# igorauad/gr-dvbs2rx

Hardware: AMD Instinct MI355X
Metric: FECFRAMEs/sec (coded Gbit/s) @ 50 LDPC iters, QPSK 1/2 normal (higher is better)
Workload: dtype int8; 1 GPU; QPSK 1/2 normal FECFRAME (DVB_S2_TABLE_B4, N=64800), 50 LDPC iterations cap, batch=4096 frames per GPU, group G=32, input=noise; frames_per_gpu=4096, max_trials=50, group_size=32, parallelism=frames sharded over 1 GPU(s), no collective

## Files before the change

### gr-dvbs2rx_amd/csrc/ldpc_kernel.hpp

```cpp
#pragma once
#include <hip/hip_runtime.h>
#include <cstdint>
#include "demap_math.hpp"
#include "ldpc_launch.h"
#include "ldpc_prims.hpp"
#include "ldpc_node_plain.hpp"
#include "ldpc_node_packed.hpp"
#include "ldpc_node_hazard.hpp"

namespace dvbs2 {

#define DVBS2_DEG_CASE(D) case D: if constexpr (D >= 3 && D <= DMAX && D > DMAX - 8) { \
        { if (layer0) check_node<(D >= 3 ? D : 3), true, false, false, TC>(lds_all, ent, jj, lb, mw, nm); else { if constexpr (!kPure) check_node<(D >= 3 ? D : 3), false, false, false, TC>(lds_all, ent, jj, lb, mw, nm); } } } else DVBS2_NM_CLEAR break;
#define DVBS2_DEG_SWITCH switch (deg) { DVBS2_DEGREES_3_32(DVBS2_DEG_CASE) default: DVBS2_NM_CLEAR break; }

#define DVBS2_V2_CASE(D) case D: if constexpr (D >= 3 && D <= DMAX && D > DMAX - 8) { check_node_v2<(D >= 3 ? D : 3), DMAX, TC>(ent, jj + lb, mw, nm, prefetch); } else DVBS2_NM_CLEAR break;
#define DVBS2_V2_SWITCH switch (deg) { DVBS2_DEGREES_3_32(DVBS2_V2_CASE) default: DVBS2_NM_CLEAR break; }
#define DVBS2_NM_CLEAR { _Pragma("unroll") for (int w_ = 0; w_ < MW; w_++) nm[w_] = 0u; }
#define DVBS2_RUN_CASE(D) case D - 2: if constexpr (D >= 3 && D <= DMAX && D > DMAX - 8) { run(std::integral_constant<int, (D >= 3 ? D : 3)>{}); } break;

#define DVBS2_CHAIN_CASE(D) case D: if constexpr (D >= 4 && D <= DMAX && D > DMAX - 8) { check_node_chain_v2<(D >= 4 ? D : 4), DMAX, TC>(ent, jj, jj + lb, work, block, mw, nm, htab16, hb_ctr, hb_epoch, hb_lane); } break;
#define DVBS2_CHAIN_SWITCH switch (deg) { DVBS2_DEGREES_4_32(DVBS2_CHAIN_CASE) default: break; }

#define DVBS2_HAZ_NODE(D, NCV, ...) \
// ... 135 lines not shown
            if (dm.mode == 1) {
                const float scalar = qpsk_scalar(N0);
                for (int sidx = tid; sidx < dm.n_syms; sidx += kHalf) {
                    const float2 v = src[sidx];
                    put(2 * sidx, qpsk_llr(v.x, scalar)); put(2 * sidx + 1, qpsk_llr(v.y, scalar));
                }
            } else {
                const float dp = psk8_dist_prec(N0);
                for (int sidx = tid; sidx < dm.n_syms; sidx += kHalf) {
                    const float2 v = src[sidx];
                    int8_t b0, b1, b2;
                    psk8_llr(v.x, v.y, dm.rr, dm.ri, dp, b0, b1, b2);
                    put(dm.ra0 + sidx, b0); put(dm.ra1 + sidx, b1); put(dm.ra2 + sidx, b2);
                }
            }
        } else if (fresh) {
            const uint2* src = reinterpret_cast<const uint2*>(llr_in + (size_t)f * N);
            for (int c = tid; c < N / 8; c += kHalf) {
                uint2 v = src[c];
                if constexpr (!TC) { v.x ^= 0x80808080u; v.y ^= 0x80808080u; }
                const int n = 8 * c;
                if (n < K) *reinterpret_cast<lds_v2u_t*>(lds + n) = (v2u32){ v.x, v.y };
                else {
                    int r = n - K;
                    int jq = r / q, iq = r - jq * q;
#pragma unroll
                    for (int b = 0; b < 8; b++) {
                        lds[K + kM * iq + jq] = (uint8_t)((b < 4 ? v.x >> (8 * b) : v.y >> (8 * (b - 4))) & 0xffu);
                        if (++iq == q) { iq = 0; ++jq; }
                    }
                }
            }
        } else {
            it = iters[f];
            if (it >= tgt) finished = true;
            else {
                const uint2* src = reinterpret_cast<const uint2*>(state + (size_t)f * N);
                for (int c = tid; c < N / 8; c += kHalf) { const uint2 v = src[c]; *reinterpret_cast<lds_v2u_t*>(lds + 8 * c) = (v2u32){ v.x ^ kObState, v.y ^ kObState }; }
            }
        }
    }
    const bool untouched = finished;
    if (tid == 0) { flags[0] = 0; flags[2] = 0; flags[3] = 0; flags[1] = finished ? 1 : 0; flags[4] = 0; }
    constexpr bool soft_bar = SOFT;
    volatile lds_i32_t* hb_ctr = soft_bar ? flags + 4 : nullptr;
    int hb_epoch = 0;
    const int hb_lane = lane;
    __syncthreads();
    TSTAMP(tB); tm_load = tB - tA;

    uint32_t* msg_base = msgs + (size_t)(have_frame ? f : 0) * q * MW * kMsgStride;
    const __amdgpu_buffer_rsrc_t mrs = __builtin_amdgcn_make_buffer_rsrc(msg_base, 0, q * MW * kMsgStride * 4, 0x00020000);
    constexpr int kLayerBytes = MW * kMsgStride * 4;
#define MSG_LD(soff, w, r4) __builtin_amdgcn_raw_buffer_load_b32(mrs, (r4), (soff) + (w) * (kMsgStride * 4), 0)
#define MSG_ST(v, soff, w, r4) __builtin_amdgcn_raw_buffer_store_b32((v), mrs, (r4), (soff) + (w) * (kMsgStride * 4), 0)
    auto msg_load = [&](uint32_t* dst, int soff, int r4) {
#pragma unroll
        for (int w = 0; w < MW; w++) dst[w] = MSG_LD(soff, w, r4);
    };
    auto msg_store = [&](const uint32_t* src, int soff, int r4) {
#pragma unroll
        for (int w = 0; w < MW; w++) MSG_ST(src[w], soff, w, r4);
    };
    auto take_msgs = [&](uint32_t* mw, uint32_t* pre, bool zero, uint32_t zero_word, int next, int r4) {
#pragma unroll
        for (int w = 0; w < MW; w++) mw[w] = pre[w];
        if (zero) {
            asm volatile("" ::: "memory");
#pragma unroll
            for (int w = 0; w < MW; w++) mw[w] = zero_word;
        } else msg_load(pre, next, r4);
    };
    bool is_good = false;

    for (;;) {
        TSTAMP(tS0);
        const bool need_synd = !finished && ((stop_on_good & 1) || it >= tgt);
        if (need_synd && active) {
            const int i0 = it % q;
            const uint32_t* rec = recs + (size_t)i0 * RS;
            const int deg = (int)(rec[0] & 0xffu) + 2;
            uint32_t x = 0, z = 0;
            constexpr bool kPretestChunk = DMAX != 16 && !(DMAX == 32 && SOFT);
            if constexpr (kPretestChunk) {
            for (int k0 = 0; k0 < deg; k0 += 4) {
                uint32_t e[8], v[4];
#pragma unroll
                for (int u = 0; u < 8; u++) e[u] = rec[4 + 2 * k0 + u];
#pragma unroll
                for (int u = 0; u < 4; u++) {
                    const int a0 = tid + (int)e[2 * u] - ((uint32_t)tid < e[2 * u + 1] ? 0 : kM);
                    v[u] = (uint32_t)lds[k0 + u < deg ? a0 : tid];
                }
#pragma unroll
                for (int u = 0; u < 4; u++) {
                    uint32_t w = v[u] ^ (TC ? 0x80u : 0x00u);
                    if (i0 == 0 && k0 + u == deg - 1 && tid == 0) w = 0x81u;
                    if (k0 + u < deg) { x ^= w; z |= (w == 0x80u); }
                }
            }
            } else
            for (int k = 0; k < deg; k++) {
                const int a0 = tid + (int)rec[4 + 2 * k] - ((uint32_t)tid < rec[5 + 2 * k] ? 0 : kM);
                uint32_t v = (uint32_t)lds[a0] ^ (TC ? 0x80u : 0x00u);
                if (i0 == 0 && k == deg - 1 && tid == 0) v = 0x81u;
                x ^= v;
                z |= (v == 0x80u);
            }
            const int bad_pre = (int)((((x >> 7) ^ (uint32_t)deg) & 1u) | z);
            if (__ballot(bad_pre) != 0 && lane == 0) flags[2] = 1;
        }
        lds_barrier();
        const bool need_full = need_synd && flags[2] == 0;
        if (tid == 0) flags[3] = need_full ? 1 : 0;
        lds_barrier();
        const bool full_any = flags[3] != 0 || (!soft_bar && !SOLO && other_flags[3] != 0);
        if (full_any) {
        if (need_full) {
            {
                const int zero = syndrome_sign_vectors(lds, sv, N, tid, TC);
                if (__ballot(zero != 0) != 0 && lane == 0) flags[0] = 1;
            }
        }
        TSTAMP(tC); tm_s1 += tC - tS0;
// ... 7 lines not shown
        lds_barrier();
        if (need_full) {
            int bad = 0;
            for (int item = tid; item < q * 12; item += kHalf) {
                const int i = item / 12, w = item - 12 * i;
                const uint32_t* rec = recs + (size_t)i * RS;
                const int deg = (int)(rec[0] & 0xffu) + 2;
                uint32_t e0[DMAX], e1[DMAX];
#pragma unroll
                for (int k = 0; k < DMAX; k++) { e0[k] = rec[4 + 2 * k]; e1[k] = rec[5 + 2 * k]; }
                uint32_t acc = 0;
#pragma unroll
                for (int k = 0; k < DMAX; k++) {
                    if (k < deg) {
                        const int rot = kM - (int)e1[k];
                        const int g360 = (int)e0[k] - rot;
                        const int t0 = wrap360(32 * w + rot);
                        const lds_u32_t* p = sv + (g360 / kM) * kSvWords + (t0 >> 5);
                        uint32_t x = __funnelshift_r(p[0], p[1], t0 & 31);
                        if (i == 0 && k == deg - 1 && w == 0) x &= ~1u;
                        acc ^= x;
                    }
                }
                if (w == 11) acc &= 0xffu;
                bad |= acc != 0;
            }
            if (__ballot(bad) != 0 && lane == 0) flags[0] = 1;
        }
        lds_barrier();
        }
        if (need_synd) is_good = need_full && flags[0] == 0;
        const bool gs = (stop_on_good & 5) == 5;
        if (!finished && (it >= tgt || (!gs && (stop_on_good & 1) && is_good))) finished = true;
        lds_barrier();
        if (wave_u == 0) {
            int fin = finished ? 1 : 0;
            if (gs && !finished) {
                const uint32_t* hd = recs - kRecHeaderWords;
                const int* iters0 = reinterpret_cast<const int*>(((unsigned long long)hd[1] << 32) | hd[0]);
                int* status = reinterpret_cast<int*>(((unsigned long long)hd[3] << 32) | hd[2]);
                const int G = (int)hd[4];
                const int g = f / G;
                fin = group_decide(status + (iters - iters0) + g * G, min(G, n_frames - g * G), f - g * G, it, is_good, lane, (int)hd[5]) != 0;
            }
            if (tid == 0) { flags[0] = 0; flags[2] = 0; flags[1] = fin; }
        }
        lds_only_barrier();
        if (gs) finished = flags[1] != 0;
        TSTAMP(tS1); tm_synd += tS1 - tS0;
        if (finished && (soft_bar || SOLO || other_flags[1])) break;

        const bool work = __builtin_amdgcn_readfirstlane(finished ? 0 : 1) != 0;
        const int row = tid < kM ? tid : kM - 1;
        const int row4 = row * 4;
        const bool zero_msgs = __builtin_amdgcn_readfirstlane(it) == 0;
        unsigned long long* const hz_ph = (TIMING && tdbg && f == 0 && (tid == 0 || tid == 320)) ? tdbg + (size_t)n_frames * 48 + 256 + (tid ? 16 : 0) : nullptr;
        uint32_t pre[MW];
        constexpr bool kWaitStore = !SOFT;
        if (work) {
#pragma unroll
            for (int w = 0; w < MW; w++) {
                pre[w] = zero_msgs ? 0x80808080u : MSG_LD(0, w, row4);
            }
        }
        constexpr bool kRun = V2 && DMAX <= 8;
        constexpr int kPfSmallMaxDmax = 8;
        constexpr int PF = DMAX <= kPfSmallMaxDmax ? 1 : 2 * DMAX;
        static_assert(!kRun || PF == 1, "the run loop takes over whole records fetched ahead into scalar registers");
        const uint32_t* wr = V2 ? wrecs + (size_t)wave_u * rec_stride_wave(DMAX) : recs;
        uint32_t nhdr = wr[0], nw1 = wr[1];
        uint32_t nent[2 * DMAX];
#pragma unroll
        for (int k = 0; k < 2 * DMAX; k += PF) nent[k] = wr[4 + k];
        DVBS2_WAIT_VM0();
        asm volatile("" : "+s"(nhdr), "+s"(nw1), "+s"(nent[0]));
        for (int i = 0; i < q; i++) {
            if constexpr (kRun) {
                if (work && !zero_msgs && i + 1 < q && (nhdr & kRecPacked) && (nhdr >> kRecBlockShift) >= (uint32_t)kM) {
                    auto run = [&](auto degc) {
                        constexpr int D = decltype(degc)::value;
                        constexpr uint32_t kKeyMask = (~0u << kRecBlockShift) | kRecPacked | 0xffu;
                        const uint32_t key = nhdr & kKeyMask;
                        uint32_t ha = nhdr, hb, ea[2 * DMAX], eb[2 * DMAX], pb[MW];
#pragma unroll
                        for (int k = 0; k < 2 * DMAX; k++) ea[k] = nent[k];
                        const uint32_t* nrec = wr + (size_t)(i + 1) * RSW;
                        int sa = i * kLayerBytes, sb;
                        const int s_last = (q - 1) * kLayerBytes;
#define DVBS2_RUN_TRIP(H, E, P, S, NH, NE, NP, NS) { \
                            TSTAMP(tA); \
                            NS = S + kLayerBytes; \
                            if (__builtin_expect((H & (1u << kRecSyncShift)) != 0u, 1)) lds_barrier(); \
                            asm volatile("" ::: "memory"); \
                            NH = nrec[0]; \
                            _Pragma("unroll") for (int k = 0; k < 2 * DMAX; k++) NE[k] = nrec[4 + k]; \
                            nrec += RSW; \
                            TSTAMP(tB); tm_bar += tB - tA; \
                            uint32_t nm[MW]; \
                            _Pragma("unroll") for (int w = 0; w < MW; w++) NP[w] = __builtin_amdgcn_raw_buffer_load_b32(mrs, row4 + w * (kMsgStride * 4), NS, 0); \
                            check_node_v2<D, DMAX, TC>(E, row + lb, P, nm, 0); \
                            DVBS2_WAIT_VM0(); \
                            _Pragma("unroll") for (int w = 0; w < MW; w++) __builtin_amdgcn_raw_buffer_store_b32(nm[w], mrs, row4 + w * (kMsgStride * 4), S, 0); \
                            TSTAMP(tC); tm_body += tC - tB; \
                            if (TIMING && tdbg && f == 0 && tid == 0) tdbg[(size_t)n_frames * 48 + S / kLayerBytes] += tC - tA; }
                        auto run_ends = [&](uint32_t h, int s) {
                            if (__builtin_expect((h & kKeyMask) != key, 0)) return true;
                            asm volatile("");
                            return (bool)__builtin_expect(s >= s_last, 0);
                        };
                        for (;;) {
                            DVBS2_RUN_TRIP(ha, ea, pre, sa, hb, eb, pb, sb)
                            if (run_ends(hb, sb)) {
                                nhdr = hb;
#pragma unroll
                                for (int k = 0; k < 2 * DMAX; k++) nent[k] = eb[k];
#pragma unroll
                                for (int w = 0; w < MW; w++) pre[w] = pb[w];
                                i = sa / kLayerBytes;
                                break;
                            }
                            DVBS2_RUN_TRIP(hb, eb, pb, sb, ha, ea, pre, sa)
                            if (run_ends(ha, sa)) {
                                nhdr = ha;
#pragma unroll
                                for (int k = 0; k < 2 * DMAX; k++) nent[k] = ea[k];
                                i = sb / kLayerBytes;
                                break;
                            }
                        }
#undef DVBS2_RUN_TRIP
                    };
                    switch (nhdr & 0xffu) { DVBS2_DEGREES_3_7(DVBS2_RUN_CASE) DVBS2_RUN_CASE(8) default: break; }
                    continue;
                }
            }
            const uint32_t hdr = nhdr;
            uint32_t ent[2 * DMAX];
#pragma unroll
            for (int k = 0; k < 2 * DMAX; k++) ent[k] = (PF <= 2 * DMAX - 1 && k % PF == 0) ? nent[k] : wr[(size_t)i * RSW + 4 + k];
            const int inext = i + 1 < q ? i + 1 : 0;
            const uint32_t* nrec = wr + (size_t)inext * RSW;
            auto prefetch = [&](uint32_t after) {
                const uint32_t* p = nrec; (void)after;
                nhdr = p[0];
                if constexpr (PF <= 2 * DMAX - 1) {
#pragma unroll
                    for (int k = 0; k < 2 * DMAX; k += PF) nent[k] = p[4 + k];
                }
            };
            constexpr int kPabMaxDmax = 8;
            constexpr bool kPab = DMAX <= kPabMaxDmax;
            if constexpr (!kPab) prefetch(0u);
            const int deg = (int)(hdr & 0xffu) + 2;
            const int nc = (int)((hdr >> 8) & 0xfu);
            lds_u32_t* htab = ((hdr >> 12) & 1u) ? sv : nullptr;
            const int block = (int)(hdr >> 16);
            int block2 = 0;
            if constexpr (HZ2 || (kTlc<DMAX, HZ2> && !SOFT && MINW == 1)) { if (block < kM) block2 = (int)wr[(size_t)i * RSW + 2]; }
            const bool layer0 = (i == 0);
            const int mso = i * kLayerBytes;
            TSTAMP(tA);
            if (hdr & 0x8000u) lds_barrier();
            if constexpr (kPab) { asm volatile("" ::: "memory"); prefetch(0u); }
            TSTAMP(tB); tm_bar += tB - tA;
            if (block >= kM) {
                if (work) {
                    const int jj = row;
                    const bool v2 = V2 && ((hdr >> 13) & 1u);
                    uint32_t mw[MW], nm[MW];
                    take_msgs(mw, pre, zero_msgs, v2 ? 0u : 0x80808080u, inext * kLayerBytes, row4);
                    if constexpr (V2) { if (v2) { DVBS2_V2_SWITCH } else DVBS2_DEG_SWITCH } else DVBS2_DEG_SWITCH
                    DVBS2_WAIT_VM0();
                    msg_store(nm, mso, row4);
                }
                TSTAMP(tC); tm_body += tC - tB;
                if (TIMING && tdbg && f == 0 && tid == 0) tdbg[(size_t)n_frames * 48 + i] += tC - tA;
            } else {
                if (nc != kHazardWalk) {
                    const int jj = row;
                    const bool hv2 = V2 && ((hdr >> 13) & 1u);
                    uint32_t mw[MW], nm[MW];
#pragma unroll
                    for (int w = 0; w < MW; w++) mw[w] = (work && !zero_msgs) ? pre[w] : (hv2 ? 0u : 0x80808080u);
                    if (work && i + 1 < q && !zero_msgs) msg_load(pre, mso + kLayerBytes, row4);
                    const bool hvp = V2 && v2p_class(DMAX) && ((hdr >> 14) & 1u);
                    if constexpr (V2 && DMAX <= 16) {
                        if (hv2) {
                            lds_u32_t* htab16 = lds_align16<lds_u32_t>(sv);
                            DVBS2_CHAIN_SWITCH
                        } else DVBS2_HAZ_SWITCH
                    } else if constexpr (V2 && v2p_class(DMAX)) { if (hvp) { DVBS2_HAZP_SWITCH } else DVBS2_HAZ_SWITCH }
                    else DVBS2_HAZ_SWITCH
                    DVBS2_WAIT_VM0();
                    if (work) msg_store(nm, mso, row4);
                } else {
                    if (!finished && wave == 0) {
                        const int chunk = block < 64 ? block : 64;
                        for (int start = 0; start < kM; start += chunk) {
                            const int jj = start + lane;
                            if (lane < chunk && jj < kM) {
                                uint32_t mw[MW], nm[MW];
#pragma unroll
                                for (int w = 0; w < MW; w++) mw[w] = zero_msgs ? 0x80808080u : MSG_LD(mso, w, jj * 4);
                                DVBS2_DEG_SWITCH
#pragma unroll
                                for (int w = 0; w < MW; w++) MSG_ST(nm[w], mso, w, jj * 4);
                            }
                        }
                    }
                    lds_barrier();
                    if (work && i + 1 < q && !zero_msgs) msg_load(pre, mso + kLayerBytes, row4);
                    DVBS2_WAIT_VM0();
                }
                TSTAMP(tC); tm_conf += tC - tB;
                if (TIMING && tdbg && f == 0 && tid == 0) tdbg[(size_t)n_frames * 48 + i] += tC - tA;
            }
        }
        TSTAMP(tA);
        lds_barrier();
        TSTAMP(tB); tm_bar += tB - tA; tm_sweep += tB - tS1;
        if (!finished) it++;
    }
    if (TIMING && tdbg && lane == 0 && have_frame) {
        unsigned long long* o = tdbg + ((size_t)f * 6 + wave) * 8;
        o[0] = tm_load; o[1] = tm_synd; o[2] = tm_sweep; o[3] = tm_bar; o[4] = tm_body; o[5] = tm_conf; o[6] = (unsigned long long)it; o[7] = tm_s1;
    }

    if (have_frame && !untouched) {
        if (tid == 0) { iters[f] = it; good[f] = is_good ? 1 : 0; }
        uint2* dst = reinterpret_cast<uint2*>(state + (size_t)f * N);
        for (int c = tid; c < N / 8; c += kHalf) { const v2u32 v = *reinterpret_cast<const lds_v2u_t*>(lds + 8 * c); dst[c] = make_uint2(v.x ^ kObState, v.y ^ kObState); }
    }
    if constexpr (SOLO) {
        if (tid == 0) __hip_atomic_fetch_add(cu_slots + solo_slot, solo_pat ? -0x10000 : -1, __ATOMIC_RELAXED, __HIP_MEMORY_SCOPE_AGENT);
    }
}

}
```

### gr-dvbs2rx_amd/csrc/ldpc_layout.h

```cpp
#pragma once
#include <cstddef>
#include <cstdint>

namespace dvbs2 {

constexpr int kM = 360;
constexpr int kMsgStride = 384;
constexpr int kSvWords = 14;

constexpr int rec_stride(int dmax) { return 2 * dmax + 4; }
constexpr int rec_stride_wave(int dmax) { return 2 * dmax + 12; }
constexpr int kRecNcShift = 8;
constexpr uint32_t kRecChain = 1u << 12;
constexpr uint32_t kRecPacked = 1u << 13;
constexpr uint32_t kRecPackedHazard = 1u << 14;
constexpr int kRecSyncShift = 15;
constexpr int kRecBlockShift = 16;
constexpr int kFlagSoftBarrier = 2;
constexpr int kFlagGroupSync = 4;
constexpr int kFlagPrSharedSv = 8;
constexpr int kRecHeaderWords = 8;
constexpr int kGroupSpinMax = 1 << 12;
constexpr int kChainMaxBlock = 180;
constexpr int kChainScratchWords = (kM + kChainMaxBlock) * 5 + 4;
constexpr int sv_area_words(int N) { return (N / kM) * kSvWords > kChainScratchWords ? (N / kM) * kSvWords : kChainScratchWords; }
constexpr size_t half_lds_bytes(int N) { return ((size_t)N + (size_t)sv_area_words(N) * 4 + 32 + 15) / 16 * 16; }
constexpr size_t pr_half_bytes(int K) { return ((size_t)K + kM + 15) / 16 * 16; }
constexpr size_t pr_lds_bytes(int N, int K, bool shared_sv = false) { return 2 * pr_half_bytes(K) + (shared_sv ? 1 : 2) * (size_t)(N / kM) * kSvWords * 4 + 64; }

constexpr bool tlc_class(int dmax) { return dmax == 16 || dmax == 24 || dmax == 32; }
constexpr bool v2p_class(int dmax) { return dmax >= 20; }
constexpr bool v2_pure_class(int dmax) { return dmax >= 32; }
constexpr int v2_nfix(int dmax) { return dmax == 32 ? 10 : dmax / 4; }

constexpr int lane_chain_words(int block) { return (kM + block) + (kM + block + 3) / 4; }
constexpr int kLaneChainMaxDeg = 28;
constexpr int kMaxHazard = 8;
constexpr int kMaxHazardHz2 = 12;
constexpr int kMaxHazard12Dmax = 28;
constexpr int kHazardWalk = 15;

constexpr int kCuSlots = 16 * 8 * 2 * 16;

enum class LdpcBuild : uint8_t {
    plain,
    packed,
    solo,
    packed_solo,
    hz2,
    soft,
    packed_soft,
    dense,
    pr,
    pr_w1,
    pr_packed,
};
constexpr int kLdpcBuilds = (int)LdpcBuild::pr_packed + 1;
constexpr bool is_solo(LdpcBuild b) { return b == LdpcBuild::solo || b == LdpcBuild::packed_solo; }
constexpr int kSoloMaxDmax = 16;

// ... 2 lines not shown
```

### gr-dvbs2rx_amd/csrc/ldpc_node_packed.hpp

```cpp
#pragma once
#include "ldpc_prims.hpp"

namespace dvbs2 {

typedef short v2s16 __attribute__((ext_vector_type(2)));
typedef unsigned short v2u16 __attribute__((ext_vector_type(2)));
__device__ __forceinline__ v2s16 as_v2s(uint32_t x) { return __builtin_bit_cast(v2s16, x); }
__device__ __forceinline__ uint32_t as_u32(v2s16 x) { return __builtin_bit_cast(uint32_t, x); }
__device__ __forceinline__ void lds_wr_hi(int a, uint32_t v) { *reinterpret_cast<lds_byte_t*>((size_t)(uint32_t)a) = (uint8_t)(v >> 16); }

__device__ __forceinline__ uint32_t msg_pair16(const uint32_t* mw, int j)
{
    const uint32_t w = mw[j >> 1];
    return (j & 1) ? (w & 0xff00ff00u) : __builtin_amdgcn_perm(w, 0u, 0x060c040cu);
}
template <int NP>
__device__ __forceinline__ void msg_pack16(const uint32_t* R , uint32_t* nm)
{
#pragma unroll
    for (int w = 0; w < (NP + 1) / 2; w++)
        nm[w] = (2 * w + 1 < NP) ? ((R[2 * w] >> 8) | R[2 * w + 1]) : (R[2 * w] >> 8);
}
template <int NP, bool ODD>
__device__ __forceinline__ void msg_pack16_hb(uint32_t* R, uint32_t* nm)
{
#pragma unroll
    for (int w = 0; w < (NP + 1) / 2; w++) {
        const bool two = 2 * w + 1 < NP;
        const bool pad_lo = ODD && !two, pad_hi = ODD && two && 2 * w + 1 == NP - 1;
        const uint32_t sel = 0x01u | (two ? 0x05u : 0x0cu) << 8 | (pad_lo ? 0x0cu : 0x03u) << 16 | ((two && !pad_hi) ? 0x07u : 0x0cu) << 24;
        nm[w] = __builtin_amdgcn_perm(two ? R[2 * w + 1] : 0u, R[2 * w], sel);
    }
}

__device__ __forceinline__ v2s16 swap16(v2s16 x) { return __builtin_shufflevector(x, x, 1, 0); }
template <int NP>
__device__ __forceinline__ void two_smallest_pk(const v2s16* a, v2s16& m0, v2s16& m1)
{
    static_assert(NP >= 2, "two pairs at least");
    constexpr int NS = (NP + 1) / 2;
    v2s16 lo[NS], hi[NS];
#pragma unroll
    for (int k = 0; k < NS; k++) {
        if (2 * k + 1 < NP) { lo[k] = __builtin_elementwise_min(a[2 * k], a[2 * k + 1]); hi[k] = __builtin_elementwise_max(a[2 * k], a[2 * k + 1]); }
        else { lo[k] = a[2 * k]; hi[k] = (v2s16){ 0x7fff, 0x7fff }; }
    }
#pragma unroll
    for (int w = 1; w < NS; w *= 2) {
#pragma unroll
        for (int k = 0; k + w < NS; k += 2 * w) {
            const bool lone = (NP & 1) && k + w == NS - 1;
            const v2s16 l = __builtin_elementwise_min(lo[k], lo[k + w]), x = __builtin_elementwise_max(lo[k], lo[k + w]);
            hi[k] = __builtin_elementwise_min(x, lone ? hi[k] : __builtin_elementwise_min(hi[k], hi[k + w]));
            lo[k] = l;
        }
    }
    const v2s16 s0 = swap16(lo[0]);
    m0 = __builtin_elementwise_min(lo[0], s0);
    m1 = __builtin_elementwise_min(__builtin_elementwise_max(lo[0], s0), __builtin_elementwise_min(hi[0], swap16(hi[0])));
}

template <bool TC>
__device__ __forceinline__ void pair_out(v2s16 d, v2s16 a, v2s16 B1p, uint32_t Tt, uint32_t tm, uint32_t& nl, uint32_t& R)
{
    const v2s16 c = __builtin_elementwise_min(a, B1p);
    const uint32_t sg = as_u32(d >> (v2s16){ 15, 15 });
    uint32_t cs;
    asm("v_bitop3_b32 %0, %1, %2, %3 bitop3:0x96" : "=v"(cs) : "v"(as_u32(c)), "v"(sg), "v"(tm));
    const v2s16 out = as_v2s(Tt ^ sg) - as_v2s(cs);
    const uint32_t sum = as_u32(__builtin_elementwise_add_sat(d, out)) ^ kObPair<TC>;
    asm("v_lshrrev_b32 %0, 8, %1" : "=v"(nl) : "v"(sum));
    R = as_u32(__builtin_elementwise_min(__builtin_elementwise_max(out, (v2s16){ -32 * 256, -32 * 256 }), (v2s16){ 31 * 256, 31 * 256 }));
}

template <int DEG, int DMAX, bool TC, class Prefetch>
__device__ __forceinline__ void check_node_v2(const uint32_t* ent ,
                                              int jjb, const uint32_t* mw, uint32_t* nm, Prefetch prefetch_next_record)
{
    constexpr int NP = (DEG + 1) / 2;
    constexpr int NFIX = v2_nfix(DMAX) < DEG - 2 ? v2_nfix(DMAX) : DEG - 2;
    constexpr bool ODD = (DEG & 1) != 0;
    __builtin_amdgcn_s_setprio(0);
    int ad[DEG];
    auto addresses = [&]() {
#pragma unroll
        for (int k = 0; k < DEG; k++) ad[k] = jjb + (int)ent[k];
#pragma unroll
        for (int k = 0; k < NFIX; k++) ad[k] = fix_wrap(ad[k], ent[DMAX + 2 * k], ent[DMAX + 2 * k + 1]);
    };
    addresses();
    int Lb[DEG];
#pragma unroll
    for (int k = 0; k < DEG; k++) Lb[k] = lds_rd(ad[k]);
    v2s16 d[NP], a[NP];
    uint32_t sx = 0;
#pragma unroll
    for (int j = 0; j < NP; j++) {
        const uint32_t M = msg_pair16(mw, j);
        const uint32_t hi = (ODD && j == NP - 1) ? (TC ? 0x00u : 0x80u) : (uint32_t)Lb[2 * j + 1];
        const uint32_t L = __builtin_amdgcn_perm(hi, (uint32_t)Lb[2 * j], 0x040c000cu) ^ kObPair<TC>;
        d[j] = __builtin_elementwise_sub_sat(as_v2s(L), as_v2s(M));
        sx ^= as_u32(d[j]);
        a[j] = __builtin_elementwise_max(d[j], __builtin_elementwise_sub_sat(as_v2s(0u), d[j]));
    }
    __builtin_amdgcn_s_setprio(1);
    (void)prefetch_next_record;
    if (ODD) a[NP - 1] = as_v2s(as_u32(a[NP - 1]) | 0x7fff0000u);
    v2s16 m0, m1;
    two_smallest_pk<NP>(a, m0, m1);
    const int n0 = (int)(as_u32(m0) & 0x7f00u), n1 = (int)(as_u32(m1) & 0x7f00u);
    const int n0m = (int)__builtin_elementwise_sub_sat((uint32_t)n0, 256u), n1m = (int)__builtin_elementwise_sub_sat((uint32_t)n1, 256u);
    const int B1 = n0 + n1m - n0m, T = n1m + n0;
    const uint32_t tm = (uint32_t)((int)(sx ^ (sx << 16)) >> 31);
    const v2s16 B1p = { (short)B1, (short)B1 };
    const uint32_t Tt = __builtin_amdgcn_perm((uint32_t)T, (uint32_t)T, 0x01000100u) ^ tm;
    uint32_t R[NP];
#pragma unroll
    for (int j = 0; j < NP; j++) {
        uint32_t nl;
        pair_out<TC>(d[j], a[j], B1p, Tt, tm, nl, R[j]);
        lds_wr(ad[2 * j], (int)nl);
        if (!(ODD && j == NP - 1)) lds_wr_hi(ad[2 * j + 1], nl);
    }
    __builtin_amdgcn_s_setprio(3);
    msg_pack16_hb<NP, ODD>(R, nm);
}

__device__ __forceinline__ float as_f32(uint32_t x) { return __builtin_bit_cast(float, x); }
__device__ __forceinline__ float vmed3_f32(float a, float b, float c) { return __builtin_amdgcn_fmed3f(a, b, c); }
__device__ __forceinline__ float byte1_f32(uint32_t x) { return (float)((x >> 8) & 0xffu); }

template <int DEG, int DMAX, bool TC>
__device__ __forceinline__ void check_node_chain_v2(const uint32_t* ent , int jj, int jjb, bool work, int B,
                                                    const uint32_t* mw, uint32_t* nm, lds_u32_t* tab ,
                                                    volatile lds_i32_t* hb_ctr, int& hb_epoch, const int hb_lane)
{
    constexpr int NP = (DEG + 1) / 2;
    constexpr int NFIXH = (v2_nfix(DMAX) + 2) < DEG - 2 ? (v2_nfix(DMAX) + 2) : DEG - 2;
    constexpr bool ODD = (DEG & 1) != 0;
    constexpr bool KEEP_AD = DEG <= 16;
    lds_v4f_t* rec = reinterpret_cast<lds_v4f_t*>(tab);
    lds_f32_t* logv = reinterpret_cast<lds_f32_t*>(tab) + 4 * (kM + kChainMaxBlock);
    const bool head = work && jj < B, body = work && jj >= B;
    const bool middle = body && jj + B < kM;
    int LbX = 0x80;
    int ad[DEG];
    v2s16 d[NP], a[NP];
    uint32_t sxp = 0;
    int p0 = 0x7fff, p1 = 0x7fff;
    int Pm = 0;
    float c = 0.f;
    __builtin_amdgcn_s_setprio(0);
    auto addresses = [&]() {
#pragma unroll
        for (int k = 0; k < DEG; k++) ad[k] = jjb + (int)ent[k];
#pragma unroll
        for (int k = 0; k < NFIXH; k++) ad[k] = fix_wrap(ad[k], ent[DMAX + 2 * k], ent[DMAX + 2 * k + 1]);
    };
    auto pair0 = [&](int LbX, int LbY) {
        const uint32_t L = __builtin_amdgcn_perm((uint32_t)LbY, (uint32_t)LbX, 0x040c000cu) ^ kObPair<TC>;
        const uint32_t M = msg_pair16(mw, 0);
        d[0] = __builtin_elementwise_sub_sat(as_v2s(L), as_v2s(M));
        a[0] = __builtin_elementwise_max(d[0], __builtin_elementwise_sub_sat(as_v2s(0u), d[0]));
    };
    if (work) {
        addresses();
        int Lb[DEG];
#pragma unroll
        for (int k = 2; k < DEG; k++) Lb[k] = lds_rd(ad[k]);
        int LbY = 0x80;
        if (head) { LbX = lds_rd(ad[0]); LbY = lds_rd(ad[1]); }
        else if (middle) LbX = lds_rd(ad[0]);
#pragma unroll
        for (int j = 1; j < NP; j++) {
            const uint32_t M = msg_pair16(mw, j);
// ... 107 lines not shown
```

### gr-dvbs2rx_amd/csrc/ldpc_plan.cpp

```cpp
#include "ldpc_plan.h"
#include <algorithm>
#include <cstdlib>
#include <cstring>

namespace dvbs2 {

LdpcOverrides LdpcOverrides::from_env()
{
    auto get = [](const char* name) -> std::optional<int> { if (const char* e = getenv(name)) return atoi(e); return std::nullopt; };
    LdpcOverrides o;
    o.pr = get("DVBS2_PR"); o.pr_w1 = get("DVBS2_PR_W1"); o.pr_v2 = get("DVBS2_PR_V2"); o.dense = get("DVBS2_DENSE"); o.hz2 = get("DVBS2_HZ2");
    o.solo = get("DVBS2_SOLO"); o.soft_barrier = get("DVBS2_SOFT_BARRIER"); o.v2 = get("DVBS2_V2"); o.v2p = get("DVBS2_V2P");
    o.group_sync = get("DVBS2_GROUP_SYNC"); o.group_spin_max = get("DVBS2_GROUP_SPIN_MAX"); o.resolve_rounds = get("DVBS2_RESOLVE_ROUNDS");
    o.timing = getenv("DVBS2_TIMING") != nullptr;
    return o;
}

namespace {
bool pick(const std::optional<int>& o, bool rule) { return o ? *o != 0 : rule; }

struct Choice {
    std::string error;
    bool pr = false, pr_w1 = false, pr_v2 = false, dense = false, hz2 = false, solo = false, soft_bar = false;
    bool packed = false;
// ... 171 lines not shown
            chain_order = pair_orientation(entry(s, L, 0), entry(s, L, 1), L.block);
        for (int w = 0; chain_order >= 0 && w < 6; w++)
            if ((int)split_wave(s, L, nullptr, 2, w).mixed.size() > v2_nfix(dmax)) chain_order = -1;
        const bool chain2 = chain_order >= 0;
        const int ncv = lr.nc[i];
        const bool v2p = c.packed && c.v2p_on && v2p_class(dmax) && hazard && !chain2 && (ncv == 2 || ncv == 4 || ncv == 8) && (int)L.cnt >= ncv;
        const bool packed_layer = i > 0 && (hazard ? chain2 || v2p : c.packed || (c.pr_v2 && i != s.q - 1 && L.cnt + 2 >= 5));
        for (int w = 0; w < 6; w++) {
            uint32_t* rec = &wr[((size_t)i * 6 + w) * RSW];
            std::copy(lr.recs.begin() + (size_t)i * RS, lr.recs.begin() + (size_t)(i + 1) * RS, rec);
            if (!packed_layer) continue;
            const WaveSplit sp = v2p ? split_wave(s, L, lr.order[i].data(), ncv, w) : split_wave(s, L, nullptr, chain2 ? 2 : 0, w);
            const int nfix = v2p ? std::min(dmax / 2, (int)L.cnt) - ncv : std::min(v2_nfix(dmax), (int)L.cnt);
            if (!chain2 && (int)sp.mixed.size() > nfix) continue;
            std::fill(rec + 4, rec + RSW, 0u);
            rec[0] |= kRecPacked | (v2p ? kRecPackedHazard : 0u);
            const int lo = 64 * w;
            int slot = 0;
            auto put = [&](int k, bool mixed) {
                const LdpcEntry& e = entry(s, L, k);
                const int thr = 360 - (int)e.rot;
                const uint32_t S0 = (uint32_t)e.base + e.rot;
                uint32_t off = S0;
                if (mixed || lo >= thr) off = S0 - 360u;
                rec[4 + slot] = off;
                if (mixed) {
                    unsigned long long m = 0;
                    for (int l = 0; l < 64; l++) if (std::min(lo + l, 359) < thr) m |= 1ull << l;
                    rec[4 + dmax + 2 * slot] = (uint32_t)m; rec[4 + dmax + 2 * slot + 1] = (uint32_t)(m >> 32);
                }
                slot++;
            };
            auto put_ordered = [&](int k) { put(k, is_mixed(entry(s, L, k), w)); };
            if (chain2) { put_ordered(chain_order); put_ordered(1 - chain_order); }
            if (v2p) for (int k = 0; k < ncv; k++) put_ordered(lr.order[i][k]);
            for (int k : sp.mixed) put(k, true);
            for (int k : sp.plain) put(k, false);
            put(L.cnt, false);
            put(L.cnt + 1, false);
        }
    }
    return wr;
}

bool has_unpacked_record(const LdpcSchedule& s, const std::vector<uint32_t>& wr, int RSW, int* layer, int* wave)
{
    for (int i = 1; i < s.q; i++)
        for (int w = 0; w < 6; w++) {
            const uint32_t h0 = wr[((size_t)i * 6 + w) * RSW];
            if (!(h0 & kRecPacked) || (s.layers[i].block < 360 && !(h0 & kRecPackedHazard))) { *layer = i; *wave = w; return true; }
        }
    return false;
}
}

LdpcPlan plan_ldpc(const LdpcSchedule& s, const char* table_name, int group_size, const LdpcOverrides& ov)
{
    LdpcPlan p;
    Choice c = select_build(s, table_name, ov);
    if (!c.error.empty()) { p.error = c.error; return p; }
    const LayerRecords lr = layer_records(s, c);
    p.wrecs = wave_records(s, c, lr);
    const int RSW = rec_stride_wave(c.dmax);
    int bad_layer = 0, bad_wave = 0;
    if (c.packed && v2_pure_class(c.dmax) && (!c.v2p_on || has_unpacked_record(s, p.wrecs, RSW, &bad_layer, &bad_wave))) {
        c.packed = false;
        p.wrecs = wave_records(s, c, lr);
    }
    if (c.packed && v2_pure_class(c.dmax) && has_unpacked_record(s, p.wrecs, RSW, &bad_layer, &bad_wave)) {
        p.error = "internal: a (layer, wave) record of a pure packed build is not in the packed format (layer " + std::to_string(bad_layer) + ", wave " + std::to_string(bad_wave) + ")";
        return p;
    }
    p.recs = lr.recs;
    p.build = build_of(c);
    p.pr = c.pr; p.pr_shared_sv = c.pr_shared_sv; p.dmax = c.dmax; p.words_per_check = c.words_per_check;
    p.gsync_on = group_size <= 64 && pick(ov.group_sync, true);
    if (p.gsync_on) p.resolve_rounds = 0;
    if (ov.group_spin_max) p.spin_max = std::max(0, *ov.group_spin_max);
    if (ov.resolve_rounds) p.resolve_rounds = std::max(0, std::min(8, *ov.resolve_rounds));
    static const char* const kSuffix[kLdpcBuilds] = { ">", ", packed>", ", solo>", ", packed, solo>", ", hz2>", ", soft>", ", packed, soft>", ", dense>",
                                                      "", "<w1>", "<packed>" };
    p.kernel_name = std::string(c.pr ? "ldpc_layered_pr_kernel" : "ldpc_layered_kernel<" + std::to_string(c.dmax)) + kSuffix[(int)p.build];
    p.solo_lds_bytes = half_lds_bytes(s.N);
    p.lds_bytes = c.pr ? pr_lds_bytes(s.N, s.K, c.pr_shared_sv) : 2 * p.solo_lds_bytes;
    return p;
}

}
```

### gr-dvbs2rx_amd/csrc/ldpc_prims.hpp

```cpp
#pragma once
#include <hip/hip_runtime.h>
#include <cstdint>
#include "ldpc_layout.h"

#define DVBS2_WAIT_VM0() do { if (kWaitStore) { asm volatile("" ::: "memory"); __builtin_amdgcn_s_waitcnt(0x0f70); asm volatile("" ::: "memory"); } } while (0)

#define DVBS2_DEGREES_4_7(X) X(4) X(5) X(6) X(7)
#define DVBS2_DEGREES_8_32(X) X(8) \
        X(9) X(10) X(11) X(12) X(13) X(14) X(15) X(16) X(17) X(18) X(19) X(20) \
        X(21) X(22) X(23) X(24) X(25) X(26) X(27) X(28) X(29) X(30) X(31) X(32)
#define DVBS2_DEGREES_3_7(X) X(3) DVBS2_DEGREES_4_7(X)
#define DVBS2_DEGREES_4_32(X) DVBS2_DEGREES_4_7(X) DVBS2_DEGREES_8_32(X)
#define DVBS2_DEGREES_3_32(X) X(3) DVBS2_DEGREES_4_32(X)

namespace dvbs2 {

constexpr int kHalf = 384;
constexpr int kThreads = 2 * kHalf;

typedef __attribute__((address_space(3))) uint8_t lds_byte_t;
typedef __attribute__((address_space(3))) uint32_t lds_u32_t;
typedef __attribute__((address_space(3))) int lds_i32_t;
typedef __attribute__((address_space(3))) float lds_f32_t;
typedef float v4f32 __attribute__((ext_vector_type(4)));
// ... 3 lines not shown
template <class T> __device__ __forceinline__ T* lds_align16(lds_u32_t* p) { return reinterpret_cast<T*>(((uint32_t)(size_t)p + 15u) & ~15u); }
__device__ __forceinline__ int wrap360(int t) { return t >= kM ? t - kM : t; }

__device__ __forceinline__ void frame_barrier(volatile lds_i32_t* ctr, int& epoch, int lane)
{
    if (!ctr) { __syncthreads(); return; }
    epoch += 6;
    asm volatile("" ::: "memory");
    if (lane == 0) __hip_atomic_fetch_add(const_cast<lds_i32_t*>(ctr), 1, __ATOMIC_RELAXED, __HIP_MEMORY_SCOPE_WORKGROUP);
    while (*ctr - epoch < 0) __builtin_amdgcn_s_sleep(1);
    asm volatile("" ::: "memory");
}
#define lds_barrier() frame_barrier(hb_ctr, hb_epoch, hb_lane)
__device__ __forceinline__ void frame_barrier_lds(volatile lds_i32_t* ctr, int& epoch, int lane)
{
    if (ctr) { frame_barrier(ctr, epoch, lane); return; }
    asm volatile("s_waitcnt lgkmcnt(0)\n\ts_barrier" ::: "memory");
}
#define lds_only_barrier() frame_barrier_lds(hb_ctr, hb_epoch, hb_lane)

__device__ __forceinline__ int group_decide(int* st , int members, int me ,
                                            int it, bool good, int lane, int spin_max = kGroupSpinMax)
{
    const int mine = ((it + 1) << 1) | (good ? 1 : 0);
    if (lane == 0) __hip_atomic_store(st + me, mine, __ATOMIC_RELAXED, __HIP_MEMORY_SCOPE_AGENT);
    if (!good) return 0;
    for (int spin = 0;; spin++) {
        int s = mine;
        if (lane < members && lane != me) s = __hip_atomic_load(st + lane, __ATOMIC_RELAXED, __HIP_MEMORY_SCOPE_AGENT);
        const bool goes_on = s > mine || s == mine - 1;
        const bool missing = s < mine - 1;
        if (__ballot(goes_on) != 0) return 0;
        if (__ballot(missing) == 0) return 1;
        if (spin >= spin_max) return 2;
        __builtin_amdgcn_s_sleep(8);
    }
}

__device__ __forceinline__ int sat_sum_u8(int a, int b)
{
    int r;
    asm("v_add3_u32 %0, %1, %2, %3\n\tv_med3_i32 %0, %0, 0, %4" : "=&v"(r) : "v"(a), "v"(b), "s"(128), "s"(255));
    return r;
}
__device__ __forceinline__ int mag_offset(int Lb, int mb)
{
    int r;
    const int a = (int)__builtin_amdgcn_sad_u16((uint32_t)Lb, (uint32_t)mb, 0xffffffffu);
    asm("v_med3_i32 %0, %1, 0, %2" : "=v"(r) : "v"(a), "s"(126));
    return r;
}
__device__ __forceinline__ int lds_rd(int a) { return *reinterpret_cast<const lds_byte_t*>((size_t)(uint32_t)a); }
__device__ __forceinline__ void lds_wr(int a, int v) { *reinterpret_cast<lds_byte_t*>((size_t)(uint32_t)a) = (uint8_t)v; }
constexpr int kTcMaxDmax = 8;
template <bool TC> __device__ __forceinline__ int lds_rdx(int a) { const int v = lds_rd(a); return TC ? (v ^ 0x80) : v; }
template <bool TC> __device__ __forceinline__ void lds_wrx(int a, int v) { lds_wr(a, TC ? (v ^ 0x80) : v); }
template <bool TC> constexpr uint32_t kObPair = TC ? 0u : 0x80008000u;
__device__ __forceinline__ int lds_address_of(const uint8_t* p) { return (int)(uint32_t)(size_t)(const lds_byte_t*)p; }

__device__ __forceinline__ int wrap_addr(int jj, int jjb, int jjb360, uint32_t S0, uint32_t thr)
{
    int r;
    asm("v_subrev_u32 %0, %4, %1\n\t"
        "v_ashrrev_i32 %0, 31, %0\n\t"
        "v_bitop3_b32 %0, %0, %2, %3 bitop3:0xca\n\t"
        "v_add_u32 %0, %5, %0"
        : "=&v"(r) : "v"(jj), "v"(jjb), "v"(jjb360), "s"(thr), "s"(S0));
    return r;
}

__device__ __forceinline__ int vmin3_i32(int a, int b, int c) { int r; asm("v_min3_i32 %0, %1, %2, %3" : "=v"(r) : "v"(a), "v"(b), "v"(c)); return r; }
__device__ __forceinline__ int vmed3_i32(int a, int b, int c) { int r; asm("v_med3_i32 %0, %1, %2, %3" : "=v"(r) : "v"(a), "v"(b), "v"(c)); return r; }
template <int N>
__device__ __forceinline__ void two_smallest(const int* v, int& m0, int& m1)
{
    static_assert(N >= 1, "empty set");
    int k;
    if constexpr (N == 1) { m0 = v[0]; m1 = 127; k = 1; }
    else if constexpr (N == 2) { m0 = min(v[0], v[1]); m1 = max(v[0], v[1]); k = 2; }
    else { m0 = vmin3_i32(v[0], v[1], v[2]); m1 = vmed3_i32(v[0], v[1], v[2]); k = 3; }
#pragma unroll
    for (; k + 3 <= N; k += 3) {
        const int g0 = vmin3_i32(v[k], v[k + 1], v[k + 2]), g1 = vmed3_i32(v[k], v[k + 1], v[k + 2]);
        const int t = max(m0, g0);
        m0 = min(m0, g0);
        m1 = vmin3_i32(t, m1, g1);
    }
#pragma unroll
    for (; k < N; k++) { m1 = vmed3_i32(m0, m1, v[k]); m0 = min(m0, v[k]); }
}

__device__ __forceinline__ int mag_raw(int Lb, int mb) { return (int)__builtin_amdgcn_sad_u16((uint32_t)Lb, (uint32_t)mb, 0xffffffffu); }
__device__ __forceinline__ int clamp_mag(int x) { int r; asm("v_med3_i32 %0, %1, 0, %2" : "=v"(r) : "v"(x), "s"(126)); return r; }
constexpr int kMagAbsent = 0x7fff;

__device__ __forceinline__ uint32_t pack4_lo8(int a, int b, int c, int d)
{
    const uint32_t lo = __builtin_amdgcn_perm((uint32_t)b, (uint32_t)a, 0x0c0c0400u);
    const uint32_t hi = __builtin_amdgcn_perm((uint32_t)d, (uint32_t)c, 0x04000c0cu);
    return lo | hi;
}

__device__ __forceinline__ int pm_pack(int magp, int d) { return (int)__builtin_amdgcn_perm((uint32_t)magp, (uint32_t)d, 0x0c0c0400u); }
__device__ __forceinline__ int pm_inp(int pm) { return __builtin_amdgcn_sbfe(pm, 0, 8); }
__device__ __forceinline__ int pm_min_clamped(int p) { return clamp_mag((int)((uint32_t)p >> 8) - 1); }

__device__ __forceinline__ int fix_wrap(int ad, uint32_t mlo, uint32_t mhi)
{
    const unsigned long long mask = ((unsigned long long)(uint32_t)__builtin_amdgcn_readfirstlane((int)mhi) << 32) | (uint32_t)__builtin_amdgcn_readfirstlane((int)mlo);
    unsigned long long save;
    asm volatile("s_mov_b64 %1, exec\n\ts_and_b64 exec, exec, %2\n\tv_add_u32 %0, 0x168, %0\n\ts_mov_b64 exec, %1"
                 : "+v"(ad), "=&s"(save) : "s"(mask) : "scc");
    return ad;
}

}
```

Before: 155,300 frames/s.

## Carry parity-chain value in registers across run loop and pack message words as b64

In the packed run loop the parity-chain variable shared by consecutive layers is kept in a register carry instead of being written to and re-read from LDS each layer. It is flushed only when the run ends. Wrap fixups now use a select via inverse ballot, and a plan-time check verifies that the records fit the carry pattern. Separately, for MW==2 the message layout interleaves the two words per row so each row is loaded and stored with a single 64-bit buffer access instead of two strided 32-bit ones. The change adds a sync barrier at run start and new correctness assumptions about record structure.

```diff
diff --git a/gr-dvbs2rx_amd/csrc/ldpc_kernel.hpp b/gr-dvbs2rx_amd/csrc/ldpc_kernel.hpp
--- a/gr-dvbs2rx_amd/csrc/ldpc_kernel.hpp
+++ b/gr-dvbs2rx_amd/csrc/ldpc_kernel.hpp
@@ -211,24 +211,34 @@
     uint32_t* msg_base = msgs + (size_t)(have_frame ? f : 0) * q * MW * kMsgStride;
     const __amdgpu_buffer_rsrc_t mrs = __builtin_amdgcn_make_buffer_rsrc(msg_base, 0, q * MW * kMsgStride * 4, 0x00020000);
     constexpr int kLayerBytes = MW * kMsgStride * 4;
-#define MSG_LD(soff, w, r4) __builtin_amdgcn_raw_buffer_load_b32(mrs, (r4), (soff) + (w) * (kMsgStride * 4), 0)
-#define MSG_ST(v, soff, w, r4) __builtin_amdgcn_raw_buffer_store_b32((v), mrs, (r4), (soff) + (w) * (kMsgStride * 4), 0)
-    auto msg_load = [&](uint32_t* dst, int soff, int r4) {
-#pragma unroll
-        for (int w = 0; w < MW; w++) dst[w] = MSG_LD(soff, w, r4);
+    constexpr int kMsgRowBytes = msg_row_bytes(MW), kMsgWordStep = msg_word_step(MW);
+#define MSG_LD(soff, w, rm) __builtin_amdgcn_raw_buffer_load_b32(mrs, (rm), (soff) + (w) * kMsgWordStep, 0)
+#define MSG_ST(v, soff, w, rm) __builtin_amdgcn_raw_buffer_store_b32((v), mrs, (rm), (soff) + (w) * kMsgWordStep, 0)
+    auto msg_load = [&](uint32_t* dst, int soff, int rm) {
+        if constexpr (MW == 2) {
+            const v2u32 v = __builtin_amdgcn_raw_buffer_load_b64(mrs, rm, soff, 0);
+            dst[0] = v.x; dst[1] = v.y;
+        } else {
+#pragma unroll
+            for (int w = 0; w < MW; w++) dst[w] = MSG_LD(soff, w, rm);
+        }
     };
-    auto msg_store = [&](const uint32_t* src, int soff, int r4) {
-#pragma unroll
-        for (int w = 0; w < MW; w++) MSG_ST(src[w], soff, w, r4);
+    auto msg_store = [&](const uint32_t* src, int soff, int rm) {
+        if constexpr (MW == 2) {
+            __builtin_amdgcn_raw_buffer_store_b64((v2u32){ src[0], src[1] }, mrs, rm, soff, 0);
+        } else {
+#pragma unroll
+            for (int w = 0; w < MW; w++) MSG_ST(src[w], soff, w, rm);
+        }
     };
-    auto take_msgs = [&](uint32_t* mw, uint32_t* pre, bool zero, uint32_t zero_word, int next, int r4) {
+    auto take_msgs = [&](uint32_t* mw, uint32_t* pre, bool zero, uint32_t zero_word, int next, int rm) {
 #pragma unroll
         for (int w = 0; w < MW; w++) mw[w] = pre[w];
         if (zero) {
             asm volatile("" ::: "memory");
 #pragma unroll
             for (int w = 0; w < MW; w++) mw[w] = zero_word;
-        } else msg_load(pre, next, r4);
+        } else msg_load(pre, next, rm);
     };
     bool is_good = false;
 
@@ -342,7 +352,7 @@
 
         const bool work = __builtin_amdgcn_readfirstlane(finished ? 0 : 1) != 0;
         const int row = tid < kM ? tid : kM - 1;
-        const int row4 = row * 4;
+        const int rowm = row * kMsgRowBytes;
         const bool zero_msgs = __builtin_amdgcn_readfirstlane(it) == 0;
         unsigned long long* const hz_ph = (TIMING && tdbg && f == 0 && (tid == 0 || tid == 320)) ? tdbg + (size_t)n_frames * 48 + 256 + (tid ? 16 : 0) : nullptr;
         uint32_t pre[MW];
@@ -350,7 +360,7 @@
         if (work) {
 #pragma unroll
             for (int w = 0; w < MW; w++) {
-                pre[w] = zero_msgs ? 0x80808080u : MSG_LD(0, w, row4);
+                pre[w] = zero_msgs ? 0x80808080u : MSG_LD(0, w, rowm);
             }
         }
         constexpr bool kRun = V2 && DMAX <= 8;
@@ -377,6 +387,13 @@
                         const uint32_t* nrec = wr + (size_t)(i + 1) * RSW;
                         int sa = i * kLayerBytes, sb;
                         const int s_last = (q - 1) * kLayerBytes;
+                        const int rowb360 = row + lb + kM;
+                        if ((ha & (1u << kRecSyncShift)) != 0u) { lds_barrier(); ha &= ~(1u << kRecSyncShift); }
+                        uint32_t carry = (uint32_t)lds_rd(row + lb + (int)ea[D - 1]) << ((D & 1) ? 24 : 8);
+                        auto flush_parity = [&](const uint32_t* E ) {
+                            const int a = row + lb + (int)E[D - 2];
+                            if constexpr ((D & 1) != 0) lds_wr_hi(a, carry >> 8); else lds_wr(a, (int)(carry >> 8));
+                        };
 #define DVBS2_RUN_TRIP(H, E, P, S, NH, NE, NP, NS) { \
                             TSTAMP(tA); \
                             NS = S + kLayerBytes; \
@@ -387,10 +404,10 @@
                             nrec += RSW; \
                             TSTAMP(tB); tm_bar += tB - tA; \
                             uint32_t nm[MW]; \
-                            _Pragma("unroll") for (int w = 0; w < MW; w++) NP[w] = __builtin_amdgcn_raw_buffer_load_b32(mrs, row4 + w * (kMsgStride * 4), NS, 0); \
-                            check_node_v2<D, DMAX, TC>(E, row + lb, P, nm, 0); \
+                            msg_load(NP, NS, rowm); \
+                            check_node_v2<D, DMAX, TC, true>(E, row + lb, P, nm, 0, rowb360, &carry); \
                             DVBS2_WAIT_VM0(); \
-                            _Pragma("unroll") for (int w = 0; w < MW; w++) __builtin_amdgcn_raw_buffer_store_b32(nm[w], mrs, row4 + w * (kMsgStride * 4), S, 0); \
+                            msg_store(nm, S, rowm); \
                             TSTAMP(tC); tm_body += tC - tB; \
                             if (TIMING && tdbg && f == 0 && tid == 0) tdbg[(size_t)n_frames * 48 + S / kLayerBytes] += tC - tA; }
                         auto run_ends = [&](uint32_t h, int s) {
@@ -401,6 +418,7 @@
                         for (;;) {
                             DVBS2_RUN_TRIP(ha, ea, pre, sa, hb, eb, pb, sb)
                             if (run_ends(hb, sb)) {
+                                flush_parity(ea);
                                 nhdr = hb;
 #pragma unroll
                                 for (int k = 0; k < 2 * DMAX; k++) nent[k] = eb[k];
@@ -411,6 +429,7 @@
                             }
                             DVBS2_RUN_TRIP(hb, eb, pb, sb, ha, ea, pre, sa)
                             if (run_ends(ha, sa)) {
+                                flush_parity(eb);
                                 nhdr = ha;
 #pragma unroll
                                 for (int k = 0; k < 2 * DMAX; k++) nent[k] = ea[k];
@@ -458,10 +477,10 @@
                     const int jj = row;
                     const bool v2 = V2 && ((hdr >> 13) & 1u);
                     uint32_t mw[MW], nm[MW];
-                    take_msgs(mw, pre, zero_msgs, v2 ? 0u : 0x80808080u, inext * kLayerBytes, row4);
+                    take_msgs(mw, pre, zero_msgs, v2 ? 0u : 0x80808080u, inext * kLayerBytes, rowm);
                     if constexpr (V2) { if (v2) { DVBS2_V2_SWITCH } else DVBS2_DEG_SWITCH } else DVBS2_DEG_SWITCH
                     DVBS2_WAIT_VM0();
-                    msg_store(nm, mso, row4);
+                    msg_store(nm, mso, rowm);
                 }
                 TSTAMP(tC); tm_body += tC - tB;
                 if (TIMING && tdbg && f == 0 && tid == 0) tdbg[(size_t)n_frames * 48 + i] += tC - tA;
@@ -472,7 +491,7 @@
                     uint32_t mw[MW], nm[MW];
 #pragma unroll
                     for (int w = 0; w < MW; w++) mw[w] = (work && !zero_msgs) ? pre[w] : (hv2 ? 0u : 0x80808080u);
-                    if (work && i + 1 < q && !zero_msgs) msg_load(pre, mso + kLayerBytes, row4);
+                    if (work && i + 1 < q && !zero_msgs) msg_load(pre, mso + kLayerBytes, rowm);
                     const bool hvp = V2 && v2p_class(DMAX) && ((hdr >> 14) & 1u);
                     if constexpr (V2 && DMAX <= 16) {
                         if (hv2) {
@@ -482,7 +501,7 @@
                     } else if constexpr (V2 && v2p_class(DMAX)) { if (hvp) { DVBS2_HAZP_SWITCH } else DVBS2_HAZ_SWITCH }
                     else DVBS2_HAZ_SWITCH
                     DVBS2_WAIT_VM0();
-                    if (work) msg_store(nm, mso, row4);
+                    if (work) msg_store(nm, mso, rowm);
                 } else {
                     if (!finished && wave == 0) {
                         const int chunk = block < 64 ? block : 64;
@@ -491,15 +510,15 @@
                             if (lane < chunk && jj < kM) {
                                 uint32_t mw[MW], nm[MW];
 #pragma unroll
-                                for (int w = 0; w < MW; w++) mw[w] = zero_msgs ? 0x80808080u : MSG_LD(mso, w, jj * 4);
+                                for (int w = 0; w < MW; w++) mw[w] = zero_msgs ? 0x80808080u : MSG_LD(mso, w, jj * kMsgRowBytes);
                                 DVBS2_DEG_SWITCH
 #pragma unroll
-                                for (int w = 0; w < MW; w++) MSG_ST(nm[w], mso, w, jj * 4);
+                                for (int w = 0; w < MW; w++) MSG_ST(nm[w], mso, w, jj * kMsgRowBytes);
                             }
                         }
                     }
                     lds_barrier();
-                    if (work && i + 1 < q && !zero_msgs) msg_load(pre, mso + kLayerBytes, row4);
+                    if (work && i + 1 < q && !zero_msgs) msg_load(pre, mso + kLayerBytes, rowm);
                     DVBS2_WAIT_VM0();
                 }
                 TSTAMP(tC); tm_conf += tC - tB;
diff --git a/gr-dvbs2rx_amd/csrc/ldpc_layout.h b/gr-dvbs2rx_amd/csrc/ldpc_layout.h
--- a/gr-dvbs2rx_amd/csrc/ldpc_layout.h
+++ b/gr-dvbs2rx_amd/csrc/ldpc_layout.h
@@ -6,6 +6,8 @@
 
 constexpr int kM = 360;
 constexpr int kMsgStride = 384;
+constexpr int msg_row_bytes(int mw) { return mw == 2 ? 8 : 4; }
+constexpr int msg_word_step(int mw) { return mw == 2 ? 4 : kMsgStride * 4; }
 constexpr int kSvWords = 14;
 
 constexpr int rec_stride(int dmax) { return 2 * dmax + 4; }
diff --git a/gr-dvbs2rx_amd/csrc/ldpc_node_packed.hpp b/gr-dvbs2rx_amd/csrc/ldpc_node_packed.hpp
--- a/gr-dvbs2rx_amd/csrc/ldpc_node_packed.hpp
+++ b/gr-dvbs2rx_amd/csrc/ldpc_node_packed.hpp
@@ -61,7 +61,7 @@
 }
 
 template <bool TC>
-__device__ __forceinline__ void pair_out(v2s16 d, v2s16 a, v2s16 B1p, uint32_t Tt, uint32_t tm, uint32_t& nl, uint32_t& R)
+__device__ __forceinline__ void pair_out(v2s16 d, v2s16 a, v2s16 B1p, uint32_t Tt, uint32_t tm, uint32_t& nl, uint32_t& R, uint32_t* sum_out = nullptr)
 {
     const v2s16 c = __builtin_elementwise_min(a, B1p);
     const uint32_t sg = as_u32(d >> (v2s16){ 15, 15 });
@@ -70,12 +70,14 @@
     const v2s16 out = as_v2s(Tt ^ sg) - as_v2s(cs);
     const uint32_t sum = as_u32(__builtin_elementwise_add_sat(d, out)) ^ kObPair<TC>;
     asm("v_lshrrev_b32 %0, 8, %1" : "=v"(nl) : "v"(sum));
+    if (sum_out) *sum_out = sum;
     R = as_u32(__builtin_elementwise_min(__builtin_elementwise_max(out, (v2s16){ -32 * 256, -32 * 256 }), (v2s16){ 31 * 256, 31 * 256 }));
 }
 
-template <int DEG, int DMAX, bool TC, class Prefetch>
+template <int DEG, int DMAX, bool TC, bool RUN = false, class Prefetch>
 __device__ __forceinline__ void check_node_v2(const uint32_t* ent ,
-                                              int jjb, const uint32_t* mw, uint32_t* nm, Prefetch prefetch_next_record)
+                                              int jjb, const uint32_t* mw, uint32_t* nm, Prefetch prefetch_next_record, int jjb360 = 0 ,
+                                              uint32_t* carry = nullptr )
 {
     constexpr int NP = (DEG + 1) / 2;
     constexpr int NFIX = v2_nfix(DMAX) < DEG - 2 ? v2_nfix(DMAX) : DEG - 2;
@@ -83,6 +85,13 @@
     __builtin_amdgcn_s_setprio(0);
     int ad[DEG];
     auto addresses = [&]() {
+        if constexpr (RUN) {
+#pragma unroll
+            for (int k = 0; k < DEG; k++)
+                if (k != DEG - 2) ad[k] = (k < NFIX ? wrap_base(jjb, jjb360, ent[DMAX + 2 * k], ent[DMAX + 2 * k + 1]) : jjb) + (int)ent[k];
+            ad[DEG - 2] = 0;
+            return;
+        }
 #pragma unroll
         for (int k = 0; k < DEG; k++) ad[k] = jjb + (int)ent[k];
 #pragma unroll
@@ -91,14 +100,17 @@
     addresses();
     int Lb[DEG];
 #pragma unroll
-    for (int k = 0; k < DEG; k++) Lb[k] = lds_rd(ad[k]);
+    for (int k = 0; k < DEG - (RUN ? 2 : 0); k++) Lb[k] = lds_rd(ad[k]);
+    if constexpr (RUN) { Lb[DEG - 2] = lds_rd_at<kM>(ad[DEG - 1]); Lb[DEG - 1] = 0; }
     v2s16 d[NP], a[NP];
     uint32_t sx = 0;
 #pragma unroll
     for (int j = 0; j < NP; j++) {
         const uint32_t M = msg_pair16(mw, j);
         const uint32_t hi = (ODD && j == NP - 1) ? (TC ? 0x00u : 0x80u) : (uint32_t)Lb[2 * j + 1];
-        const uint32_t L = __builtin_amdgcn_perm(hi, (uint32_t)Lb[2 * j], 0x040c000cu) ^ kObPair<TC>;
+        const uint32_t Lp = !(RUN && j == NP - 1) ? __builtin_amdgcn_perm(hi, (uint32_t)Lb[2 * j], 0x040c000cu)
+                            : ODD ? __builtin_amdgcn_perm(hi, *carry, 0x040c030cu) : __builtin_amdgcn_perm(*carry, (uint32_t)Lb[2 * j], 0x050c000cu);
+        const uint32_t L = Lp ^ kObPair<TC>;
         d[j] = __builtin_elementwise_sub_sat(as_v2s(L), as_v2s(M));
         sx ^= as_u32(d[j]);
         a[j] = __builtin_elementwise_max(d[j], __builtin_elementwise_sub_sat(as_v2s(0u), d[j]));
@@ -118,9 +130,9 @@
 #pragma unroll
     for (int j = 0; j < NP; j++) {
         uint32_t nl;
-        pair_out<TC>(d[j], a[j], B1p, Tt, tm, nl, R[j]);
-        lds_wr(ad[2 * j], (int)nl);
-        if (!(ODD && j == NP - 1)) lds_wr_hi(ad[2 * j + 1], nl);
+        pair_out<TC>(d[j], a[j], B1p, Tt, tm, nl, R[j], RUN && j == (DEG - 2) / 2 ? carry : nullptr);
+        if (!(RUN && 2 * j == DEG - 2)) lds_wr(ad[2 * j], (int)nl);
+        if (!(ODD && j == NP - 1) && !(RUN && 2 * j + 1 == DEG - 2)) lds_wr_hi(ad[2 * j + 1], nl);
     }
     __builtin_amdgcn_s_setprio(3);
     msg_pack16_hb<NP, ODD>(R, nm);
diff --git a/gr-dvbs2rx_amd/csrc/ldpc_plan.cpp b/gr-dvbs2rx_amd/csrc/ldpc_plan.cpp
--- a/gr-dvbs2rx_amd/csrc/ldpc_plan.cpp
+++ b/gr-dvbs2rx_amd/csrc/ldpc_plan.cpp
@@ -247,6 +247,24 @@
         }
     return false;
 }
+
+bool parity_chain_ok(const LdpcSchedule& s, const std::vector<uint32_t>& wr, int dmax, int* layer, int* wave)
+{
+    const int RSW = rec_stride_wave(dmax);
+    constexpr uint32_t kKey = (~0u << kRecBlockShift) | kRecPacked | 0xffu;
+    auto mask = [&](const uint32_t* r, int slot) { return slot < v2_nfix(dmax) ? r[4 + dmax + 2 * slot] | r[4 + dmax + 2 * slot + 1] : 0u; };
+    for (int i = 1; i + 1 < s.q; i++)
+        for (int w = 0; w < 6; w++) {
+            const uint32_t* a = &wr[((size_t)i * 6 + w) * RSW];
+            const uint32_t* b = a + (size_t)6 * RSW;
+            if (!(a[0] & kRecPacked) || (a[0] >> kRecBlockShift) < 360u) continue;
+            const int own = (int)(a[0] & 0xffu), prev = own + 1;
+            bool ok = a[4 + own] == a[4 + prev] + 360u && !mask(a, own) && !mask(a, prev);
+            if (i + 2 < s.q && (a[0] & kKey) == (b[0] & kKey)) ok = ok && b[4 + prev] == a[4 + own];
+            if (!ok) { *layer = i; *wave = w; return false; }
+        }
+    return true;
+}
 }
 
 LdpcPlan plan_ldpc(const LdpcSchedule& s, const char* table_name, int group_size, const LdpcOverrides& ov)
@@ -264,6 +282,10 @@
     }
     if (c.packed && v2_pure_class(c.dmax) && has_unpacked_record(s, p.wrecs, RSW, &bad_layer, &bad_wave)) {
         p.error = "internal: a (layer, wave) record of a pure packed build is not in the packed format (layer " + std::to_string(bad_layer) + ", wave " + std::to_string(bad_wave) + ")";
+        return p;
+    }
+    if (c.packed && !c.pr && c.dmax <= 8 && !parity_chain_ok(s, p.wrecs, c.dmax, &bad_layer, &bad_wave)) {
+        p.error = "internal: the parity slots of a packed regular record do not fit the run loop's parity carry (layer " + std::to_string(bad_layer) + ", wave " + std::to_string(bad_wave) + ")";
         return p;
     }
     p.recs = lr.recs;
diff --git a/gr-dvbs2rx_amd/csrc/ldpc_prims.hpp b/gr-dvbs2rx_amd/csrc/ldpc_prims.hpp
--- a/gr-dvbs2rx_amd/csrc/ldpc_prims.hpp
+++ b/gr-dvbs2rx_amd/csrc/ldpc_prims.hpp
@@ -79,6 +79,7 @@
 }
 __device__ __forceinline__ int lds_rd(int a) { return *reinterpret_cast<const lds_byte_t*>((size_t)(uint32_t)a); }
 __device__ __forceinline__ void lds_wr(int a, int v) { *reinterpret_cast<lds_byte_t*>((size_t)(uint32_t)a) = (uint8_t)v; }
+template <int OFF> __device__ __forceinline__ int lds_rd_at(int a) { return *(reinterpret_cast<const lds_byte_t*>((size_t)(uint32_t)a) + OFF); }
 constexpr int kTcMaxDmax = 8;
 template <bool TC> __device__ __forceinline__ int lds_rdx(int a) { const int v = lds_rd(a); return TC ? (v ^ 0x80) : v; }
 template <bool TC> __device__ __forceinline__ void lds_wrx(int a, int v) { lds_wr(a, TC ? (v ^ 0x80) : v); }
@@ -140,5 +141,10 @@
                  : "+v"(ad), "=&s"(save) : "s"(mask) : "scc");
     return ad;
 }
+__device__ __forceinline__ int wrap_base(int b, int b360, uint32_t mlo, uint32_t mhi)
+{
+    const unsigned long long mask = ((unsigned long long)(uint32_t)__builtin_amdgcn_readfirstlane((int)mhi) << 32) | (uint32_t)__builtin_amdgcn_readfirstlane((int)mlo);
+    return __builtin_amdgcn_inverse_ballot_w64(mask) ? b360 : b;
+}
 
 }
```

New measurement: 159,000 frames/s (median of 6 runs). 2.4% higher.
